# piotrmwojcik/GI-GS

Measured on AMD Instinct MI355X. Metric: train-step renders/sec (fwd+bwd, G-buffer+indirect) at 800x800; PSNR vs the CPU oracle, higher is better.
Workload: dtype f32; 1 GPU; C2 (configs[1] TensoIR lego stand-in): 300k surface Gaussians, 800x800, SH deg 2, GI step=16 start=8 delta=0.0625; P=300000, N=640000, M=9, hip_graphs=on, fused_glue=on, gi_march=proj, rasterizer=whole step = 2 hand-captured hipGraphs (fwd, bwd), asynchronous binning

## Files before the change

### gi-gs_amd/csrc/api.hip

```cpp
#include <cstdarg>
#include <cstdio>
#include <cstdlib>
#include <cstring>
#include <map>
#include <algorithm>
#include <new>
#include <mutex>
#include <vector>

#include "../../include/gigs_hip.h"
#include "gigs_common.h"

namespace {

thread_local char g_err[512] = "";

int fail(int code, const char* fmt, ...) {
  va_list ap;
  va_start(ap, fmt);
  vsnprintf(g_err, sizeof(g_err), fmt, ap);
  va_end(ap);
  return code;
}

// ... 70 lines not shown
  const char* ll = getenv("GIGS_LONG_LISTS");
  o.long_lists = (ll && ll[0]) ? (ll[0] == '1' ? 1 : 0) : -1;
  o.bucket_target = std::max(256, env_int("GIGS_BUCKET_TARGET", 1536));
  o.bin_bands = std::max(0, env_int("GIGS_BIN_BANDS", 0));
  o.blend_cull = env_int("GIGS_BLEND_CULL", 1) != 0;
  o.pre_bwd_sh_skip = env_int("GIGS_PRE_BWD_SH_SKIP", 1) != 0;
  o.gi_march = 4;
  if (const char* e = getenv("GIGS_GI_MARCH")) {
    if (strcmp(e, "exact") == 0) o.gi_march = 0;
  }
  o.gi_cert = env_int("GIGS_GI_CERT", 1) != 0;
  o.gi_interleave = env_int("GIGS_GI_INTERLEAVE", 1) != 0;
  o.gi_tile_log2w = env_int("GIGS_GI_TILE_LOG2W", 3);
  if (o.gi_tile_log2w < 0 || o.gi_tile_log2w > 6) o.gi_tile_log2w = 3;
  o.gi_zero_rays = env_int("GIGS_GI_ZERO_RAYS", 0) != 0;
  o.spec_max8 = env_int("GIGS_SPEC_MAX8", 128);
  o.spec_max16 = env_int("GIGS_SPEC_MAX16", 1500);
  o.shade_lds_floats = env_int("GIGS_SHADE_LDS_FLOATS", 30 * 1024);
  o.shade_bwd_blocks = std::max(0, env_int("GIGS_SHADE_BWD_BLOCKS", 0));
  o.shade_bwd_rows = env_int("GIGS_SHADE_BWD_ROWS", 0) != 0;
  o.spec_sparse = env_int("GIGS_SPEC_SPARSE", 1) != 0;
  o.spec_sparse_permille = env_int("GIGS_SPEC_SPARSE_PERMILLE", 37);
  if (o.spec_sparse_permille < 0 || o.spec_sparse_permille > 1000) o.spec_sparse_permille = 37;
  return o;
}
const gigs::Ctx& ctx_of(const gigs_ctx* c) { return c ? *reinterpret_cast<const gigs::Ctx*>(c) : gigs::default_ctx(); }

struct ProfRec { int stage; hipEvent_t a, b; };
std::mutex g_prof_mu;
bool g_prof_on = false;
std::vector<ProfRec> g_prof_recs;
std::vector<hipEvent_t> g_prof_pool;

hipEvent_t prof_event() {
  if (!g_prof_pool.empty()) {
    hipEvent_t e = g_prof_pool.back();
    g_prof_pool.pop_back();
    return e;
  }
  hipEvent_t e;
  hipEventCreate(&e);
  return e;
}

struct StageScope {
  hipStream_t s;
// ... 82 lines not shown
  gigs::ImageState s = gigs::ImageState::fromChunk(p, N, T);
  const void* ptrs[] = {s.final_T, s.n_contrib, s.ranges, s.tile_order};
  if (which < 0 || which >= 4) return -1;
  return (long long)((const char*)ptrs[which] - base);
}

gigs_ctx* gigs_ctx_create(void) {
  gigs::Ctx* c = new (std::nothrow) gigs::Ctx(gigs::default_ctx());
  if (!c) fail(GIGS_ERR_ALLOC, "gigs_ctx_create: out of host memory");
  return reinterpret_cast<gigs_ctx*>(c);
}
void gigs_ctx_destroy(gigs_ctx* ctx) { delete reinterpret_cast<gigs::Ctx*>(ctx); }

int gigs_ctx_get_options(const gigs_ctx* ctx, gigs_options* out) {
  if (!out || out->struct_bytes < (int)sizeof(gigs_options)) return fail(GIGS_ERR_INVALID, "gigs_ctx_get_options: set struct_bytes = sizeof(gigs_options)");
  const gigs::Options& o = ctx_of(ctx).opt;
  out->struct_bytes = (int)sizeof(gigs_options);
  out->binning_legacy = o.binning_legacy; out->bucket_max_mean = o.bucket_max_mean; out->long_lists = o.long_lists;
  out->bucket_target = o.bucket_target; out->bin_bands = o.bin_bands; out->blend_cull = o.blend_cull; out->pre_bwd_sh_skip = o.pre_bwd_sh_skip;
  out->gi_march = o.gi_march; out->gi_cert = o.gi_cert; out->gi_interleave = o.gi_interleave;
  out->gi_tile_log2w = o.gi_tile_log2w; out->gi_zero_rays = o.gi_zero_rays; out->spec_max8 = o.spec_max8;
  out->spec_max16 = o.spec_max16; out->shade_lds_floats = o.shade_lds_floats; out->shade_bwd_blocks = o.shade_bwd_blocks;
  out->shade_bwd_rows = o.shade_bwd_rows; out->spec_sparse = o.spec_sparse; out->spec_sparse_permille = o.spec_sparse_permille;
  return 0;
}
int gigs_ctx_set_options(gigs_ctx* ctx, const gigs_options* in) {
  if (!ctx) return fail(GIGS_ERR_INVALID, "gigs_ctx_set_options: the default context is immutable, create one");
  if (!in || in->struct_bytes < (int)sizeof(gigs_options)) return fail(GIGS_ERR_INVALID, "gigs_ctx_set_options: set struct_bytes = sizeof(gigs_options)");
  if (in->gi_march != 0 && in->gi_march != 4) return fail(GIGS_ERR_INVALID, "gi_march must be 0 (exact) or 4 (proj)");
  if (in->gi_tile_log2w < 0 || in->gi_tile_log2w > 6) return fail(GIGS_ERR_INVALID, "gi_tile_log2w must be 0..6");
  if (in->long_lists < -1 || in->long_lists > 1) return fail(GIGS_ERR_INVALID, "long_lists must be -1, 0 or 1");
  if (in->bucket_target < 256 || in->bucket_max_mean < 0 || in->bin_bands < 0 || in->bin_bands > 64)
    return fail(GIGS_ERR_INVALID, "bucket_target >= 256, bucket_max_mean >= 0, 0 <= bin_bands <= 64");
  if (in->spec_max8 < 0 || in->spec_max16 < in->spec_max8) return fail(GIGS_ERR_INVALID, "0 <= spec_max8 <= spec_max16");
  if (in->shade_lds_floats < 0 || in->shade_bwd_blocks < 0) return fail(GIGS_ERR_INVALID, "shade_lds_floats, shade_bwd_blocks >= 0");
  if (in->spec_sparse_permille < 0 || in->spec_sparse_permille > 1000) return fail(GIGS_ERR_INVALID, "0 <= spec_sparse_permille <= 1000");
  gigs::Options& o = reinterpret_cast<gigs::Ctx*>(ctx)->opt;
  o.binning_legacy = in->binning_legacy != 0; o.bucket_max_mean = in->bucket_max_mean; o.long_lists = in->long_lists;
  o.bucket_target = in->bucket_target; o.bin_bands = in->bin_bands; o.blend_cull = in->blend_cull != 0; o.pre_bwd_sh_skip = in->pre_bwd_sh_skip != 0;
  o.gi_march = in->gi_march; o.gi_cert = in->gi_cert != 0; o.gi_interleave = in->gi_interleave != 0;
  o.gi_tile_log2w = in->gi_tile_log2w; o.gi_zero_rays = in->gi_zero_rays != 0; o.spec_max8 = in->spec_max8;
  o.spec_max16 = in->spec_max16; o.shade_lds_floats = in->shade_lds_floats; o.shade_bwd_blocks = in->shade_bwd_blocks;
  o.shade_bwd_rows = in->shade_bwd_rows != 0; o.spec_sparse = in->spec_sparse != 0; o.spec_sparse_permille = in->spec_sparse_permille;
  return 0;
}
int gigs_ctx_set_reuse_binning(gigs_ctx* ctx, int on) {
  if (!ctx) return fail(GIGS_ERR_INVALID, "gigs_ctx_set_reuse_binning: the default context is immutable, create one");
  reinterpret_cast<gigs::Ctx*>(ctx)->reuse_binning = on != 0;
  return 0;
}
int gigs_ctx_set_split_sh(gigs_ctx* ctx, const float* sh_rest) {
  if (!ctx) return fail(GIGS_ERR_INVALID, "gigs_ctx_set_split_sh: the default context is immutable, create one");
  reinterpret_cast<gigs::Ctx*>(ctx)->sh_rest = sh_rest;
  return 0;
}
int gigs_ctx_set_materials_only(gigs_ctx* ctx, void* violations) {
  if (!ctx) return fail(GIGS_ERR_INVALID, "gigs_ctx_set_materials_only: the default context is immutable, create one");
  reinterpret_cast<gigs::Ctx*>(ctx)->materials_only = reinterpret_cast<unsigned*>(violations);
  return 0;
}
int gigs_ctx_set_blend_begin_event(gigs_ctx* ctx, void* hip_event) {
  if (!ctx) return fail(GIGS_ERR_INVALID, "gigs_ctx_set_blend_begin_event: the default context is immutable, create one");
  reinterpret_cast<gigs::Ctx*>(ctx)->blend_begin_event = hip_event;
  return 0;
}

// ... 499 lines not shown
```

### gi-gs_amd/csrc/gigs_common.h

```cpp
#pragma once
#include <hip/hip_runtime.h>
#include <stdint.h>

#define GIGS_BLOCK_X 16
#define GIGS_BLOCK_Y 16
#define GIGS_TILE (GIGS_BLOCK_X * GIGS_BLOCK_Y)
#define GIGS_BREC_F4 5
#define GIGS_GREC 20

namespace gigs {

struct v3 { float x, y, z; };
struct v4 { float x, y, z, w; };

__device__ __forceinline__ v3 operator+(v3 a, v3 b) { return {a.x + b.x, a.y + b.y, a.z + b.z}; }
__device__ __forceinline__ v3 operator-(v3 a, v3 b) { return {a.x - b.x, a.y - b.y, a.z - b.z}; }
__device__ __forceinline__ v3 operator*(v3 a, float s) { return {a.x * s, a.y * s, a.z * s}; }
__device__ __forceinline__ float dot3(v3 a, v3 b) { return a.x * b.x + a.y * b.y + a.z * b.z; }
__device__ __forceinline__ v3 cross3(v3 a, v3 b) {
  return {a.y * b.z - a.z * b.y, a.z * b.x - a.x * b.z, a.x * b.y - a.y * b.x};
}
__device__ __forceinline__ v3 normalize3(v3 v) {
  float inv = 1.0f / sqrtf(dot3(v, v));
  return v * inv;
// ... 164 lines not shown
  S::fromChunk(p, a...);
  return reinterpret_cast<size_t>(p) + kAlign;
}

struct Options {
  int binning_legacy;
  int bucket_max_mean;
  int long_lists;
  int bucket_target;
  int bin_bands;
  int blend_cull;
  int pre_bwd_sh_skip;
  int gi_march;
  int gi_cert;
  int gi_interleave;
  int gi_tile_log2w;
  int gi_zero_rays;
  int spec_max8, spec_max16;
  int shade_lds_floats;
  int shade_bwd_blocks;
  int shade_bwd_rows;
  int spec_sparse;
  int spec_sparse_permille;
};
struct Ctx {
  Options opt;
  unsigned async_capacity;
  unsigned* async_counters;
  void* blend_begin_event;
  int reuse_binning;
  unsigned* materials_only;
  const float* sh_rest;
};
const Options& default_options();
const Ctx& default_ctx();

struct FwdArgs {
  int P, D, M, W, H;
  unsigned gx, gy;
  float focal_x, focal_y, tan_fovx, tan_fovy, scale_modifier;
  const float *means3D, *shs, *colors_precomp, *opacities, *normal, *albedo, *roughness,
      *metallic, *scales, *rotations, *cov3D_precomp, *viewmatrix, *projmatrix, *cam_pos,
      *background;
  int argmax_depth, inference;
  const float* shs_rest;
};
// ... 72 lines not shown
```

### gi-gs_amd/csrc/pbr.hip

```cpp
#include <cmath>
#include <cstdlib>
#include <cstring>
#include <map>
#include <mutex>
#include <vector>

#include "gigs_common.h"
#include "pixel_ops.h"

namespace gigs {

__device__ __forceinline__ v3 safe_normalize(v3 v) {
  const float l = sqrtf(v.x * v.x + v.y * v.y + v.z * v.z);
  return l > 0.0f ? v3{v.x / l, v.y / l, v.z / l} : v3{0, 0, 0};
}
__device__ __forceinline__ v3 cube_dir_raw(float fx, float fy, int side) {
  switch (side) {
    case 0: return {1, -fy, -fx};
    case 1: return {-1, -fy, fx};
    case 2: return {fx, 1, fy};
    case 3: return {fx, -1, -fy};
    case 4: return {fx, -fy, 1};
    default: return {-fx, -fy, -1};
  }
// ... 252 lines not shown
      const int yy = (int)(((float)i + 0.5f) * inv), xx = i - yy * wd;
      const float w = W[(size_t)base + i];
      W2[(size_t)base + i] = w >= 0.0f ? w / divisor[(s * N + ymin + yy) * N + xmin + xx] : w;
    }
  }
}

typedef float pbr_f2 __attribute__((ext_vector_type(2)));

template <int kLanes>
__device__ __forceinline__ float group_sum_last(float v) {
  v += pbr_dpp<0xb1>(v);
  v += pbr_dpp<0x4e>(v);
  if (kLanes == 8) return v + pbr_dpp<0x141>(v);
  v += pbr_dpp<0x124>(v);
  v += pbr_dpp<0x128>(v);
  if (kLanes == 64) {
    v += pbr_dpp<0x142, 0xa>(v);
    v += pbr_dpp<0x143, 0xc>(v);
  }
  return v;
}

template <bool kBackward, bool kNorm, int kLanes>
__device__ __forceinline__ void specular_apply_body(int block, int N, const float* __restrict__ src,
                                                    const float* __restrict__ bounds, const uint32_t* __restrict__ offsets,
                                                    const float* __restrict__ W, float* __restrict__ dst,
                                                    float* __restrict__ wsum_out) {
  constexpr int kPerWave = 64 / kLanes;
  constexpr int kU = 4;
  const int lane = threadIdx.x & 63;
  const int total = 6 * N * N;
  const int o_raw = (block * 4 + (threadIdx.x >> 6)) * kPerWave + lane / kLanes;
  const bool valid = o_raw < total;
  const int o = valid ? o_raw : total - 1;
  const int g = lane % kLanes;
  const int stride = (kBackward && !kNorm) ? 4 : 3;

  __shared__ int face_tab[4 * kPerWave * 20];
  int* tab = face_tab + ((threadIdx.x >> 6) * kPerWave + lane / kLanes) * 20;
  const float4* b4 = reinterpret_cast<const float4*>(bounds + 24 * (size_t)o);
  const uint32_t first = offsets[6 * (size_t)o];
  int n_all;
  {
    int wd[6], pre[7], base[6];
    pre[0] = 0;
#pragma unroll
    for (int s = 0; s < 6; ++s) {
      const float4 b = b4[s];
      const int xmin = (int)b.x, xmax = (int)b.y, ymin = (int)b.z, ymax = (int)b.w;
      const bool empty = xmin > xmax || ymin > ymax;
      wd[s] = empty ? 1 : xmax - xmin + 1;
      pre[s + 1] = pre[s] + (empty ? 0 : wd[s] * (ymax - ymin + 1));
      base[s] = empty ? 0 : (s * N + ymin) * N + xmin;
    }
    n_all = pre[6];
    if (g == 0) {
#pragma unroll
      for (int s = 0; s < 7; ++s) tab[s] = pre[s];
#pragma unroll
      for (int s = 0; s < 6; ++s) { tab[8 + s] = wd[s]; tab[14 + s] = base[s]; }
    }
// ... 85 lines not shown
  float c0 = acc01.x, c1 = acc01.y, c2 = accw2.y, wsum = accw2.x;
  c0 = group_sum_last<kLanes>(c0); c1 = group_sum_last<kLanes>(c1); c2 = group_sum_last<kLanes>(c2);
  if (!kBackward) wsum = group_sum_last<kLanes>(wsum);
  if (g == kLanes - 1 && valid) {
    if (kBackward) {
      float* q = dst + 3 * (size_t)o;
      q[0] = c0; q[1] = c1; q[2] = c2;
    } else if (kNorm) {
      float* q = dst + 3 * (size_t)o;
      q[0] = c0 / wsum; q[1] = c1 / wsum; q[2] = c2 / wsum;
      wsum_out[o] = wsum;
    } else {
      float* q = dst + 4 * (size_t)o;
      q[0] = c0; q[1] = c1; q[2] = c2; q[3] = wsum;
    }
  }
}

template <bool kBackward, bool kNorm, int kLanes>
__global__ void __launch_bounds__(256)
specular_apply_kernel(int N, const float* __restrict__ src, const float* __restrict__ bounds,
                      const uint32_t* __restrict__ offsets, const float* __restrict__ W,
                      float* __restrict__ dst, float* __restrict__ wsum_out) {
  specular_apply_body<kBackward, kNorm, kLanes>(blockIdx.x, N, src, bounds, offsets, W, dst, wsum_out);
}

struct SpecLevel {
  int N, lanes, block_begin;
  const float* src;
  const float* bounds;
  const uint32_t* offsets;
  const float* W;
  float* dst;
  float* wsum_out;
};
struct SpecLevels { int n; SpecLevel lv[8]; };

template <bool kBackward>
__global__ void __launch_bounds__(256) specular_apply_multi_kernel(SpecLevels L) {
  int k = 0;
#pragma unroll
  for (int i = 1; i < 8; i++)
    if (i < L.n && (int)blockIdx.x >= L.lv[i].block_begin) k = i;
  const SpecLevel& v = L.lv[k];
  const int block = (int)blockIdx.x - v.block_begin;
  if (v.lanes == 8) specular_apply_body<kBackward, true, 8>(block, v.N, v.src, v.bounds, v.offsets, v.W, v.dst, v.wsum_out);
  else if (v.lanes == 16) specular_apply_body<kBackward, true, 16>(block, v.N, v.src, v.bounds, v.offsets, v.W, v.dst, v.wsum_out);
  else specular_apply_body<kBackward, true, 64>(block, v.N, v.src, v.bounds, v.offsets, v.W, v.dst, v.wsum_out);
}

static int spec_lanes_for(const Options& o, int avg_window) {
  return (avg_window > 0 && avg_window <= o.spec_max8) ? 8 : (avg_window > 0 && avg_window <= o.spec_max16) ? 16 : 64;
}

template <bool kBackward, bool kNorm>
static void launch_specular_apply(const Options& o, int res, int avg_window, const float* src, const float* bounds,
                                  const uint32_t* offsets, const float* W, float* dst, float* wsum_out, hipStream_t s) {
  const int total = 6 * res * res;
  const int max8 = o.spec_max8, max16 = o.spec_max16;
  if (avg_window > 0 && avg_window <= max8) {
    const int waves = (total + 7) / 8;
    hipLaunchKernelGGL((specular_apply_kernel<kBackward, kNorm, 8>), dim3((waves + 3) / 4), dim3(256), 0, s, res, src,
                       bounds, offsets, W, dst, wsum_out);
  } else if (avg_window > 0 && avg_window <= max16) {
    const int waves = (total + 3) / 4;
    hipLaunchKernelGGL((specular_apply_kernel<kBackward, kNorm, 16>), dim3((waves + 3) / 4), dim3(256), 0, s, res, src,
                       bounds, offsets, W, dst, wsum_out);
  } else {
    hipLaunchKernelGGL((specular_apply_kernel<kBackward, kNorm, 64>), dim3((total + 3) / 4), dim3(256), 0, s, res, src,
                       bounds, offsets, W, dst, wsum_out);
  }
}

struct SparseLevel {
  int total, cap, block_begin, group_begin, N;
  int vec;
  int chunks;
  int lds;
  const float* src;
  float* dst;
  const float* bounds;
  const uint32_t* offsets;
  const float* Wfwd;
  const float* wsum;
  int* list;
};
struct SparseLevels { int n; SparseLevel lv[8]; };

constexpr int kCensusPerThread = 4;

__global__ void __launch_bounds__(256) specular_census_kernel(SparseLevels L, int* __restrict__ state) {
  int k = 0;
#pragma unroll
  for (int i = 1; i < 8; i++)
    if (i < L.n && (int)blockIdx.x >= L.lv[i].block_begin) k = i;
  const SparseLevel& v = L.lv[k];
  const int lane = threadIdx.x & 63;
  const int t0 = (((int)blockIdx.x - v.block_begin) * 256 + (int)threadIdx.x) * kCensusPerThread;
  bool nz[kCensusPerThread];
  if (v.vec && t0 + kCensusPerThread <= v.total) {
    const float4* s4 = reinterpret_cast<const float4*>(v.src + 3 * (size_t)t0);
    float4* d4 = reinterpret_cast<float4*>(v.dst + 3 * (size_t)t0);
    const float4 a = s4[0], b = s4[1], c = s4[2];
    nz[0] = a.x != 0.0f || a.y != 0.0f || a.z != 0.0f;
    nz[1] = a.w != 0.0f || b.x != 0.0f || b.y != 0.0f;
    nz[2] = b.z != 0.0f || b.w != 0.0f || c.x != 0.0f;
    nz[3] = c.y != 0.0f || c.z != 0.0f || c.w != 0.0f;
    const float4 z = {0.0f, 0.0f, 0.0f, 0.0f};
    d4[0] = z; d4[1] = z; d4[2] = z;
  } else {
#pragma unroll
    for (int j = 0; j < kCensusPerThread; j++) {
      nz[j] = false;
      if (t0 + j < v.total) {
        const float* s = v.src + 3 * (size_t)(t0 + j);
        float* d = v.dst + 3 * (size_t)(t0 + j);
        nz[j] = s[0] != 0.0f || s[1] != 0.0f || s[2] != 0.0f;
        d[0] = 0.0f; d[1] = 0.0f; d[2] = 0.0f;
      }
    }
  }
  unsigned long long m[kCensusPerThread];
  int wave_total = 0;
#pragma unroll
  for (int j = 0; j < kCensusPerThread; j++) { m[j] = __ballot(nz[j]); wave_total += __popcll(m[j]); }
  __shared__ int wave_base[5];
  const int wave = threadIdx.x >> 6;
  if (lane == 0) wave_base[wave] = wave_total;
  __syncthreads();
  if (threadIdx.x == 0) {
    const int t01 = wave_base[0] + wave_base[1], t012 = t01 + wave_base[2], all = t012 + wave_base[3];
    const int first = all ? atomicAdd(state + k, all) : 0;
    wave_base[3] = first + t012; wave_base[2] = first + t01; wave_base[1] = first + wave_base[0]; wave_base[0] = first;
  }
  __syncthreads();
  if (wave_total == 0) return;
  int base = wave_base[wave];
  const unsigned long long below = (1ull << lane) - 1ull;
#pragma unroll
  for (int j = 0; j < kCensusPerThread; j++) {
    const int slot = base + __popcll(m[j] & below);
    if (nz[j] && slot < v.cap) v.list[slot] = t0 + j;
    base += __popcll(m[j]);
  }
}

constexpr int kScatterU = 2;
constexpr int kLdsTile = 32;
constexpr int kLdsParts = 8;
constexpr int kLdsWide = 16;

__global__ void __launch_bounds__(256) specular_scatter_kernel(SparseLevels L, int* __restrict__ state) {
  const int lane = threadIdx.x & 63;
  const int group = (int)blockIdx.x * 4 + ((int)threadIdx.x >> 6);
  if (blockIdx.x == 0 && threadIdx.x < 8 && (int)threadIdx.x < L.n) {
    const int c = state[threadIdx.x];
    state[8 + threadIdx.x] = c <= L.lv[threadIdx.x].cap ? 1 : 0;
    state[16 + threadIdx.x] = c;
  }
  int k = 0;
#pragma unroll
  for (int i = 1; i < 8; i++)
    if (i < L.n && group >= L.lv[i].group_begin) k = i;
  const SparseLevel& v = L.lv[k];
  const int count = state[k];
  if (count > v.cap) return;
  if (v.lds) {
    __shared__ float img[kLdsTile * kLdsTile * 3];
    const int N = v.N, nt = (N + kLdsTile - 1) / kLdsTile, bl = (group - v.group_begin) >> 2;
    const int face = bl % 6, tile = (bl / 6) % (nt * nt), part = bl / (6 * nt * nt);
    const int tx0 = (tile % nt) * kLdsTile, ty0 = (tile / nt) * kLdsTile;
    const int tx1 = min(tx0 + kLdsTile, N) - 1, ty1 = min(ty0 + kLdsTile, N) - 1;
    const int wave = (int)threadIdx.x >> 6;
    for (int i = threadIdx.x; i < kLdsTile * kLdsTile * 3; i += 256) img[i] = 0.0f;
    __syncthreads();
    const int listed = min(count, v.cap);
    for (int slot = part + kLdsParts * wave; slot < listed; slot += kLdsParts * 4) {
      const int o = __builtin_amdgcn_readfirstlane(v.list[slot]);
      const float4* b4 = reinterpret_cast<const float4*>(v.bounds + 24 * (size_t)o);
      int before = 0, xmin = 0, xmax = -1, ymin = 0, ymax = -1;
#pragma unroll
      for (int s = 0; s < 6; ++s) {
        const float4 b = b4[s];
        const int x0 = (int)b.x, x1 = (int)b.y, y0 = (int)b.z, y1 = (int)b.w;
        const int cnt = (x0 > x1 || y0 > y1) ? 0 : (x1 - x0 + 1) * (y1 - y0 + 1);
        if (s < face) before += cnt;
        if (s == face && cnt) { xmin = x0; xmax = x1; ymin = y0; ymax = y1; }
      }
      const int ix0 = max(xmin, tx0), ix1 = min(xmax, tx1), iy0 = max(ymin, ty0), iy1 = min(ymax, ty1);
      if (ix0 > ix1 || iy0 > iy1) continue;
      const int wd = xmax - xmin + 1, iw = ix1 - ix0 + 1, ni = iw * (iy1 - iy0 + 1);
// ... 6 lines not shown
        const float w = W[(y - ymin) * wd + (x - xmin)];
        if (!(w >= 0.0f)) continue;
        float* t = img + 3 * ((y - ty0) * kLdsTile + (x - tx0));
        const float q = w / ws;
        const float v0 = q * g0, v1 = q * g1, v2 = q * g2;
        if (v0 != 0.0f) atomicAdd(t, v0);
        if (v1 != 0.0f) atomicAdd(t + 1, v1);
        if (v2 != 0.0f) atomicAdd(t + 2, v2);
      }
    }
    __syncthreads();
    const int row3 = 3 * (tx1 - tx0 + 1), cells = row3 * (ty1 - ty0 + 1);
    for (int i = threadIdx.x; i < cells; i += 256) {
      const int yy = i / row3, xc = i - yy * row3;
      const float val = img[3 * yy * kLdsTile + xc];
      if (val != 0.0f) atomicAdd(v.dst + 3 * ((size_t)(face * N + ty0 + yy) * N + tx0) + xc, val);
    }
    return;
  }
  const int slot = (group - v.group_begin) / v.chunks, chunk = (group - v.group_begin) % v.chunks;
  if (slot >= count || slot >= v.cap) return;
  const int o = __builtin_amdgcn_readfirstlane(v.list[slot]);
  const int N = v.N;
  int pre[7], wd[6], base[6];
  float inv[6];
  pre[0] = 0;
  const float4* b4 = reinterpret_cast<const float4*>(v.bounds + 24 * (size_t)o);
#pragma unroll
  for (int s = 0; s < 6; ++s) {
    const float4 b = b4[s];
    const int xmin = (int)b.x, xmax = (int)b.y, ymin = (int)b.z, ymax = (int)b.w;
    const bool empty = xmin > xmax || ymin > ymax;
    wd[s] = empty ? 1 : xmax - xmin + 1;
    inv[s] = 1.0f / (float)wd[s];
    pre[s + 1] = pre[s] + (empty ? 0 : wd[s] * (ymax - ymin + 1));
    base[s] = empty ? 0 : (s * N + ymin) * N + xmin;
  }
  const int n = pre[6];
  const float* W = v.Wfwd + v.offsets[6 * (size_t)o];
  const float ws = v.wsum[o];
  const float* g = v.src + 3 * (size_t)o;
  const float g0 = g[0], g1 = g[1], g2 = g[2];
  const int step = 64 * v.chunks;
  int from[3];
  float gch[3];
#pragma unroll
  for (int j = 0; j < 3; j++) {
    const int D = 64 * j + lane, ch = D % 3;
    from[j] = D / 3;
    gch[j] = ch == 0 ? g0 : ch == 1 ? g1 : g2;
  }
  const int ch0 = lane % 3;
  for (int c0 = 64 * chunk; c0 < n; c0 += step * kScatterU) {
    float w[kScatterU];
#pragma unroll
    for (int u = 0; u < kScatterU; u++) {
      const int c = c0 + u * step + lane;
      w[u] = c < n ? W[c] : -1.0f;
    }
#pragma unroll
    for (int u = 0; u < kScatterU; u++) {
      if (c0 + u * step >= n) break;
      const int c = c0 + u * step + lane;
      float q = -1.0f;
      int texel = 0;
      if (w[u] >= 0.0f) {
        int f = 0;
#pragma unroll
        for (int j = 1; j < 6; j++) f += c >= pre[j] ? 1 : 0;
        int f_pre = pre[0], f_wd = wd[0], f_base = base[0];
        float f_inv = inv[0];
#pragma unroll
        for (int j = 1; j < 6; j++)
          if (f == j) { f_pre = pre[j]; f_wd = wd[j]; f_base = base[j]; f_inv = inv[j]; }
        const int loc = c - f_pre;
        const int row = (int)(((float)loc + 0.5f) * f_inv);
        texel = f_base + row * N + (loc - row * f_wd);
        q = w[u] / ws;
      }
#pragma unroll
      for (int j = 0; j < 3; j++) {
        const float qq = __shfl(q, from[j]);
        const int tt = __shfl(texel, from[j]);
        const int ch = ch0 + j >= 3 ? ch0 + j - 3 : ch0 + j;
        const float val = qq * gch[j];
        if (!(qq < 0.0f) && val != 0.0f) atomicAdd(v.dst + 3 * (size_t)tt + ch, val);
      }
    }
  }
}

__global__ void __launch_bounds__(256) specular_apply_multi_bwd_sparse_kernel(SpecLevels L, int* __restrict__ state) {
  int k = 0;
#pragma unroll
  for (int i = 1; i < 8; i++)
    if (i < L.n && (int)blockIdx.x >= L.lv[i].block_begin) k = i;
  if (blockIdx.x == 0 && threadIdx.x < 8) state[threadIdx.x] = 0;
  if (state[8 + k] != 0) return;
  const SpecLevel& v = L.lv[k];
  const int block = (int)blockIdx.x - v.block_begin;
  if (v.lanes == 8) specular_apply_body<true, true, 8>(block, v.N, v.src, v.bounds, v.offsets, v.W, v.dst, v.wsum_out);
  else if (v.lanes == 16) specular_apply_body<true, true, 16>(block, v.N, v.src, v.bounds, v.offsets, v.W, v.dst, v.wsum_out);
  else specular_apply_body<true, true, 64>(block, v.N, v.src, v.bounds, v.offsets, v.W, v.dst, v.wsum_out);
}

static int spec_sparse_capacity(const Options& o, int res) {
  return (int)((long long)6 * res * res * o.spec_sparse_permille / 1000);
}

__device__ __forceinline__ int cube_face_uv(float x, float y, float z, float& u, float& v) {
  const float ax = fabsf(x), ay = fabsf(y), az = fabsf(z);
  int idx;
  float c;
  if (az > fmaxf(ax, ay)) { idx = 4; c = z; }
  else if (ay > ax) { idx = 2; c = y; y = z; }
  else { idx = 0; c = x; x = z; }
  if (c < 0.f) idx += 1;
  const float m = (1.0f / fabsf(c)) * 0.5f;
  const float m0 = (idx == 0 || idx == 5) ? -m : m;
  const float m1 = (idx != 2) ? -m : m;
  u = x * m0 + 0.5f;
  v = y * m1 + 0.5f;
  if (!isfinite(u) || !isfinite(v)) return -1;
  u = fminf(fmaxf(u, 0.f), 1.f);
  v = fminf(fmaxf(v, 0.f), 1.f);
  return idx;
// ... 823 lines not shown
  void* tok; gigs_internal_stage_begin(backward ? 17 : 16, stream, &tok);
  if (backward) hipLaunchKernelGGL(gigs::specular_apply_multi_kernel<true>, dim3(blocks), dim3(256), 0, (hipStream_t)stream, L);
  else hipLaunchKernelGGL(gigs::specular_apply_multi_kernel<false>, dim3(blocks), dim3(256), 0, (hipStream_t)stream, L);
  gigs_internal_stage_end(tok);
  PBR_CHECK_LAUNCH();
  return 0;
}

int gigs_spec_sparse_capacity(const gigs_ctx* ctx, int res) {
  if (res <= 0 || res > 4096) return gigs_internal_fail(GIGS_ERR_INVALID, "spec_sparse_capacity: bad resolution");
  return gigs::spec_sparse_capacity(*gigs_internal_options(ctx), res);
}

int gigs_specular_cubemap_multi_bwd_sparse(gigs_ctx* ctx, int n_levels, const gigs_spec_level* levels,
                                           const float* const* weights_fwd, const float* const* wsum, int* state,
                                           int* lists, void* stream) {
  const gigs::Options& o = *gigs_internal_options(ctx);
  if (!o.spec_sparse) return gigs_specular_cubemap_multi_w(ctx, n_levels, levels, 1, stream);
  if (n_levels <= 0 || n_levels > 8 || !levels || !weights_fwd || !wsum || !state || !lists)
    return gigs_internal_fail(GIGS_ERR_INVALID, "specular_cubemap_multi_bwd_sparse: bad argument");
  gigs::SpecLevels L;
  gigs::SparseLevels S;
  L.n = S.n = n_levels;
  int blocks = 0, census_blocks = 0, groups = 0;
  size_t list_begin = 0;
  for (int i = 0; i < n_levels; i++) {
    const gigs_spec_level& a = levels[i];
    if (a.res <= 0 || a.res > 4096 || !a.src || !a.bounds || !a.offsets || !a.weights || !a.dst || !weights_fwd[i] || !wsum[i])
      return gigs_internal_fail(GIGS_ERR_INVALID, "specular_cubemap_multi_bwd_sparse: bad level");
    gigs::SpecLevel& v = L.lv[i];
    v.N = a.res; v.lanes = gigs::spec_lanes_for(o, a.avg_window); v.block_begin = blocks;
    v.src = a.src; v.bounds = a.bounds; v.offsets = a.offsets; v.W = a.weights; v.dst = a.dst; v.wsum_out = a.wsum;
    const int total = 6 * a.res * a.res;
    const int waves = v.lanes == 64 ? total : (total + (64 / v.lanes) - 1) / (64 / v.lanes);
    blocks += (waves + 3) / 4;
    gigs::SparseLevel& q = S.lv[i];
    q.total = total; q.cap = gigs::spec_sparse_capacity(o, a.res); q.block_begin = census_blocks; q.group_begin = groups; q.N = a.res;
    q.vec = ((((uintptr_t)a.src) | ((uintptr_t)a.dst)) & 15) == 0;
    q.src = a.src; q.dst = a.dst; q.bounds = a.bounds; q.offsets = a.offsets; q.Wfwd = weights_fwd[i]; q.wsum = wsum[i];
    q.list = lists + list_begin;
    const int per_block = 256 * gigs::kCensusPerThread;
    census_blocks += (total + per_block - 1) / per_block;
    q.chunks = std::min(32, std::max(1, (std::max(1, a.avg_window) + 64 * 2 * gigs::kScatterU - 1) / (64 * 2 * gigs::kScatterU)));
    q.lds = (long long)a.avg_window * gigs::kLdsWide >= total;
    const int nt = (a.res + gigs::kLdsTile - 1) / gigs::kLdsTile;
    groups += q.lds ? 4 * 6 * nt * nt * gigs::kLdsParts : (q.cap * q.chunks + 3) / 4 * 4;
    list_begin += (size_t)q.cap;
  }
  hipStream_t s = (hipStream_t)stream;
  void* tok; gigs_internal_stage_begin(17, stream, &tok);
  hipLaunchKernelGGL(gigs::specular_census_kernel, dim3(census_blocks), dim3(256), 0, s, S, state);
  hipLaunchKernelGGL(gigs::specular_scatter_kernel, dim3(std::max(1, (groups + 3) / 4)), dim3(256), 0, s, S, state);
  hipLaunchKernelGGL(gigs::specular_apply_multi_bwd_sparse_kernel, dim3(blocks), dim3(256), 0, s, L, state);
  gigs_internal_stage_end(tok);
  PBR_CHECK_LAUNCH();
  return 0;
}

int gigs_cubemap_mip_fwd(int res_out, int channels, const float* in, float* out, void* stream) {
  if (res_out <= 0 || channels <= 0 || !in || !out) return gigs_internal_fail(GIGS_ERR_INVALID, "cubemap_mip_fwd: bad argument");
  void* tok; gigs_internal_stage_begin(16, stream, &tok);
  hipLaunchKernelGGL(gigs::cubemap_mip_fwd_kernel, dim3((6 * res_out * res_out * channels + 255) / 256), dim3(256), 0, (hipStream_t)stream, res_out, channels, in, out);
  gigs_internal_stage_end(tok);
  PBR_CHECK_LAUNCH();
  return 0;
}

int gigs_cubemap_mip_bwd(int res_out, const float* dout, float* din, void* stream) {
  if (res_out <= 0 || !dout || !din) return gigs_internal_fail(GIGS_ERR_INVALID, "cubemap_mip_bwd: bad argument");
  const int res = 2 * res_out;
  void* tok; gigs_internal_stage_begin(17, stream, &tok);
  hipLaunchKernelGGL(gigs::cubemap_mip_bwd_kernel, dim3((6 * res * res + 255) / 256), dim3(256), 0, (hipStream_t)stream, res_out, dout, din, (const float*)nullptr,
                     (const float*)nullptr);
  gigs_internal_stage_end(tok);
  PBR_CHECK_LAUNCH();
  return 0;
// ... 273 lines not shown
```

### gi-gs_amd/gigs_lib.py

```python
from __future__ import annotations

import ctypes as C
import functools
import os
import threading

_HERE = os.path.dirname(os.path.abspath(__file__))
LIB_PATH = os.environ.get("GIGS_LIB", os.path.join(_HERE, "libgigs_hip.so"))

ALLOC_FN = C.CFUNCTYPE(C.c_void_p, C.c_size_t, C.c_void_p)

_f = C.c_void_p
_i = C.c_int
_fl = C.c_float

SIGNATURES = {
    "gigs_last_error": (C.c_char_p, []),
    "gigs_build_arch": (C.c_char_p, []),
    "gigs_required_geom": (C.c_size_t, [_i]),
    "gigs_required_image": (C.c_size_t, [_i, _i]),
    "gigs_required_binning": (C.c_size_t, [_i]),
    "gigs_forward": (_i, [C.c_void_p, ALLOC_FN, C.c_void_p, ALLOC_FN, C.c_void_p, ALLOC_FN, C.c_void_p,
                          _i, _i, _i, _f, _i, _i,
                          _f, _f, _f, _f, _f, _f, _f, _f,
# ... 119 lines not shown
    "gigs_stream_delay": (_i, [C.c_uint, C.c_void_p]),
    "gigs_ctx_set_async_binning": (_i, [C.c_void_p, _i, C.c_void_p]),
    "gigs_ctx_create": (C.c_void_p, []),
    "gigs_ctx_destroy": (None, [C.c_void_p]),
    "gigs_ctx_get_options": (_i, [C.c_void_p, C.c_void_p]),
    "gigs_ctx_set_options": (_i, [C.c_void_p, C.c_void_p]),
    "gigs_profile_begin": (None, []),
    "gigs_profile_end": (_i, [C.POINTER(C.c_float), C.POINTER(C.c_int), _i]),
    "gigs_profile_stage_name": (C.c_char_p, [_i]),
}

class ShadeExt(C.Structure):
    _fields_ = [("planar", C.c_int), ("rough_scale", C.c_float), ("rough_bias", C.c_float),
                ("out_F0", C.c_void_p), ("out_linear", C.c_void_p), ("out_roughness", C.c_void_p),
                ("g_albedo_mul_a", C.c_void_p), ("g_albedo_mul_b", C.c_void_p),
                ("g_roughness_add", C.c_void_p), ("g_metallic_add", C.c_void_p),
                ("g_scale", C.c_void_p), ("lamb_mask", C.c_void_p), ("lamb_acc4", C.c_void_p)]


class Options(C.Structure):
    _fields_ = [(n, C.c_int) for n in (
        "struct_bytes", "binning_legacy", "bucket_max_mean", "long_lists", "bucket_target", "bin_bands", "blend_cull",
        "pre_bwd_sh_skip", "gi_march", "gi_cert", "gi_interleave", "gi_tile_log2w", "gi_zero_rays", "spec_max8",
        "spec_max16", "shade_lds_floats", "shade_bwd_blocks", "shade_bwd_rows", "spec_sparse", "spec_sparse_permille")]


OPTION_NAMES = tuple(n for n, _ in Options._fields_ if n != "struct_bytes")
GI_MARCHES = {0: "exact", 4: "proj"}
_GI_MARCH_VALUES = {name: value for value, name in GI_MARCHES.items()}


class SpecLevel(C.Structure):
    _fields_ = [("res", C.c_int), ("avg_window", C.c_int), ("src", C.c_void_p), ("bounds", C.c_void_p),
                ("offsets", C.c_void_p), ("weights", C.c_void_p), ("dst", C.c_void_p), ("wsum", C.c_void_p)]


class AdamGroup(C.Structure):
    _fields_ = [("param", C.c_void_p), ("grad", C.c_void_p), ("exp_avg", C.c_void_p), ("exp_avg_sq", C.c_void_p),
                ("n", C.c_longlong), ("lr", C.c_double), ("step", C.c_int)]


class ActivationRaw(C.Structure):
    _fields_ = [(n, C.c_void_p) for n in ("f_dc", "f_rest", "opacity", "normal", "albedo", "roughness", "metallic",
                                          "scaling", "rotation")]


class ActivationOut(C.Structure):
# ... 221 lines not shown
```

### include/gigs_hip.h

```cpp
#ifndef GIGS_HIP_H_
#define GIGS_HIP_H_

#include <stddef.h>
#include <stdint.h>

#ifdef __cplusplus
extern "C" {
#endif

#define GIGS_OK 0
#define GIGS_ERR_INVALID (-1)
#define GIGS_ERR_HIP (-2)
#define GIGS_ERR_ALLOC (-3)

typedef char* (*gigs_alloc_fn)(size_t nbytes, void* user);

const char* gigs_last_error(void);
const char* gigs_build_arch(void);

typedef struct gigs_ctx gigs_ctx;
typedef struct gigs_options {
  int struct_bytes;
  int binning_legacy;
  int bucket_max_mean;
  int long_lists;
  int bucket_target;
  int bin_bands;
  int blend_cull;
  int pre_bwd_sh_skip;
  int gi_march;
  int gi_cert;
  int gi_interleave;
  int gi_tile_log2w;
  int gi_zero_rays;
  int spec_max8;
  int spec_max16;
  int shade_lds_floats;
  int shade_bwd_blocks;
  int shade_bwd_rows;
  int spec_sparse;
  int spec_sparse_permille;
} gigs_options;
gigs_ctx* gigs_ctx_create(void);
void gigs_ctx_destroy(gigs_ctx* ctx);
int gigs_ctx_get_options(const gigs_ctx* ctx, gigs_options* out);
int gigs_ctx_set_options(gigs_ctx* ctx, const gigs_options* in);

size_t gigs_required_geom(int P);
size_t gigs_required_image(int width, int height);
size_t gigs_required_binning(int num_rendered);

int gigs_forward(gigs_ctx* ctx, gigs_alloc_fn geometryBuffer, void* geom_user, gigs_alloc_fn binningBuffer,
                 void* binning_user, gigs_alloc_fn imageBuffer, void* image_user, int P, int D, int M,
                 const float* background, int width, int height, const float* means3D,
                 const float* shs, const float* colors_precomp, const float* opacities,
                 const float* normal, const float* albedo, const float* roughness,
                 const float* metallic, const float* scales, float scale_modifier,
                 const float* rotations, const float* cov3D_precomp, const float* viewmatrix,
                 const float* projmatrix, const float* cam_pos, float tan_fovx, float tan_fovy,
                 int prefiltered, int argmax_depth, int inference, float* out_color,
                 float* out_opacity, float* out_depth, float* out_normal, float* out_normal_view,
                 float* out_pos, float* out_albedo, float* out_roughness, float* out_metallic,
                 int* radii, int debug, void* stream);

// ... 317 lines not shown
```

Baseline: 353.9 renders/s.

## Fuse sparse specular scatter and dense backward apply into one launch

The backward sparse specular path drops from three kernels to two. The census kernel now finalises the per-level sparse/dense decision through a last-block ticket atomic. A single fused kernel then runs both the sparse scatter groups and the dense apply blocks, each block skipping itself according to that decision. Scatter groups are reordered so LDS-tiled levels come first, and the per-object face table moves from registers into LDS. The fused path is on by default and guarded by an option. It removes one launch and its serialisation point, at the cost of a larger shared LDS buffer and a grid that holds both block types.

```diff
diff --git a/gi-gs_amd/csrc/api.hip b/gi-gs_amd/csrc/api.hip
--- a/gi-gs_amd/csrc/api.hip
+++ b/gi-gs_amd/csrc/api.hip
@@ -116,6 +116,7 @@
   o.spec_sparse = env_int("GIGS_SPEC_SPARSE", 1) != 0;
   o.spec_sparse_permille = env_int("GIGS_SPEC_SPARSE_PERMILLE", 37);
   if (o.spec_sparse_permille < 0 || o.spec_sparse_permille > 1000) o.spec_sparse_permille = 37;
+  o.spec_sparse_fused = env_int("GIGS_SPEC_SPARSE_FUSED", 1) != 0;
   return o;
 }
 const gigs::Ctx& ctx_of(const gigs_ctx* c) { return c ? *reinterpret_cast<const gigs::Ctx*>(c) : gigs::default_ctx(); }
@@ -244,6 +245,7 @@
   out->gi_tile_log2w = o.gi_tile_log2w; out->gi_zero_rays = o.gi_zero_rays; out->spec_max8 = o.spec_max8;
   out->spec_max16 = o.spec_max16; out->shade_lds_floats = o.shade_lds_floats; out->shade_bwd_blocks = o.shade_bwd_blocks;
   out->shade_bwd_rows = o.shade_bwd_rows; out->spec_sparse = o.spec_sparse; out->spec_sparse_permille = o.spec_sparse_permille;
+  out->spec_sparse_fused = o.spec_sparse_fused;
   return 0;
 }
 int gigs_ctx_set_options(gigs_ctx* ctx, const gigs_options* in) {
@@ -264,6 +266,7 @@
   o.gi_tile_log2w = in->gi_tile_log2w; o.gi_zero_rays = in->gi_zero_rays != 0; o.spec_max8 = in->spec_max8;
   o.spec_max16 = in->spec_max16; o.shade_lds_floats = in->shade_lds_floats; o.shade_bwd_blocks = in->shade_bwd_blocks;
   o.shade_bwd_rows = in->shade_bwd_rows != 0; o.spec_sparse = in->spec_sparse != 0; o.spec_sparse_permille = in->spec_sparse_permille;
+  o.spec_sparse_fused = in->spec_sparse_fused != 0;
   return 0;
 }
 int gigs_ctx_set_reuse_binning(gigs_ctx* ctx, int on) {
diff --git a/gi-gs_amd/csrc/gigs_common.h b/gi-gs_amd/csrc/gigs_common.h
--- a/gi-gs_amd/csrc/gigs_common.h
+++ b/gi-gs_amd/csrc/gigs_common.h
@@ -210,6 +210,7 @@
   int shade_bwd_rows;
   int spec_sparse;
   int spec_sparse_permille;
+  int spec_sparse_fused;
 };
 struct Ctx {
   Options opt;
diff --git a/gi-gs_amd/csrc/pbr.hip b/gi-gs_amd/csrc/pbr.hip
--- a/gi-gs_amd/csrc/pbr.hip
+++ b/gi-gs_amd/csrc/pbr.hip
@@ -298,11 +298,13 @@
   return v;
 }
 
+constexpr int kFaceTabInts(int lanes) { return 4 * (64 / lanes) * 20; }
+
 template <bool kBackward, bool kNorm, int kLanes>
 __device__ __forceinline__ void specular_apply_body(int block, int N, const float* __restrict__ src,
                                                     const float* __restrict__ bounds, const uint32_t* __restrict__ offsets,
                                                     const float* __restrict__ W, float* __restrict__ dst,
-                                                    float* __restrict__ wsum_out) {
+                                                    float* __restrict__ wsum_out, int* face_tab) {
   constexpr int kPerWave = 64 / kLanes;
   constexpr int kU = 4;
   const int lane = threadIdx.x & 63;
@@ -313,7 +315,6 @@
   const int g = lane % kLanes;
   const int stride = (kBackward && !kNorm) ? 4 : 3;
 
-  __shared__ int face_tab[4 * kPerWave * 20];
   int* tab = face_tab + ((threadIdx.x >> 6) * kPerWave + lane / kLanes) * 20;
   const float4* b4 = reinterpret_cast<const float4*>(bounds + 24 * (size_t)o);
   const uint32_t first = offsets[6 * (size_t)o];
@@ -445,7 +446,8 @@
 specular_apply_kernel(int N, const float* __restrict__ src, const float* __restrict__ bounds,
                       const uint32_t* __restrict__ offsets, const float* __restrict__ W,
                       float* __restrict__ dst, float* __restrict__ wsum_out) {
-  specular_apply_body<kBackward, kNorm, kLanes>(blockIdx.x, N, src, bounds, offsets, W, dst, wsum_out);
+  __shared__ int face_tab[kFaceTabInts(kLanes)];
+  specular_apply_body<kBackward, kNorm, kLanes>(blockIdx.x, N, src, bounds, offsets, W, dst, wsum_out, face_tab);
 }
 
 struct SpecLevel {
@@ -460,16 +462,20 @@
 struct SpecLevels { int n; SpecLevel lv[8]; };
 
 template <bool kBackward>
+__device__ __forceinline__ void specular_apply_level(const SpecLevel& v, int block, int* face_tab) {
+  if (v.lanes == 8) specular_apply_body<kBackward, true, 8>(block, v.N, v.src, v.bounds, v.offsets, v.W, v.dst, v.wsum_out, face_tab);
+  else if (v.lanes == 16) specular_apply_body<kBackward, true, 16>(block, v.N, v.src, v.bounds, v.offsets, v.W, v.dst, v.wsum_out, face_tab);
+  else specular_apply_body<kBackward, true, 64>(block, v.N, v.src, v.bounds, v.offsets, v.W, v.dst, v.wsum_out, face_tab);
+}
+
+template <bool kBackward>
 __global__ void __launch_bounds__(256) specular_apply_multi_kernel(SpecLevels L) {
   int k = 0;
 #pragma unroll
   for (int i = 1; i < 8; i++)
     if (i < L.n && (int)blockIdx.x >= L.lv[i].block_begin) k = i;
-  const SpecLevel& v = L.lv[k];
-  const int block = (int)blockIdx.x - v.block_begin;
-  if (v.lanes == 8) specular_apply_body<kBackward, true, 8>(block, v.N, v.src, v.bounds, v.offsets, v.W, v.dst, v.wsum_out);
-  else if (v.lanes == 16) specular_apply_body<kBackward, true, 16>(block, v.N, v.src, v.bounds, v.offsets, v.W, v.dst, v.wsum_out);
-  else specular_apply_body<kBackward, true, 64>(block, v.N, v.src, v.bounds, v.offsets, v.W, v.dst, v.wsum_out);
+  __shared__ int face_tab[kFaceTabInts(8)];
+  specular_apply_level<kBackward>(L.lv[k], (int)blockIdx.x - L.lv[k].block_begin, face_tab);
 }
 
 static int spec_lanes_for(const Options& o, int avg_window) {
@@ -496,7 +502,8 @@
 }
 
 struct SparseLevel {
-  int total, cap, block_begin, group_begin, N;
+  int total, cap, block_begin, N;
+  int group_begin, group_end;
   int vec;
   int chunks;
   int lds;
@@ -512,6 +519,9 @@
 
 constexpr int kCensusPerThread = 4;
 
+constexpr int kSparseTicket = 24;
+
+template <bool kFinish>
 __global__ void __launch_bounds__(256) specular_census_kernel(SparseLevels L, int* __restrict__ state) {
   int k = 0;
 #pragma unroll
@@ -555,6 +565,20 @@
     const int t01 = wave_base[0] + wave_base[1], t012 = t01 + wave_base[2], all = t012 + wave_base[3];
     const int first = all ? atomicAdd(state + k, all) : 0;
     wave_base[3] = first + t012; wave_base[2] = first + t01; wave_base[1] = first + wave_base[0]; wave_base[0] = first;
+    int one = 1;
+    asm volatile("" : "+v"(one) : "v"(first));
+    if (kFinish && __hip_atomic_fetch_add(state + kSparseTicket, one, __ATOMIC_RELAXED, __HIP_MEMORY_SCOPE_AGENT) == (int)gridDim.x - 1) {
+#pragma unroll
+      for (int l = 0; l < 8; l++) {
+        if (l < L.n) {
+          const int c = __hip_atomic_load(state + l, __ATOMIC_RELAXED, __HIP_MEMORY_SCOPE_AGENT);
+          state[8 + l] = c <= L.lv[l].cap ? 1 : 0;
+          state[16 + l] = c;
+        }
+        state[l] = 0;
+      }
+      state[kSparseTicket] = 0;
+    }
   }
   __syncthreads();
   if (wave_total == 0) return;
@@ -572,24 +596,22 @@
 constexpr int kLdsTile = 32;
 constexpr int kLdsParts = 8;
 constexpr int kLdsWide = 16;
-
-__global__ void __launch_bounds__(256) specular_scatter_kernel(SparseLevels L, int* __restrict__ state) {
+constexpr int kSparseLdsFloats = kLdsTile * kLdsTile * 3;
+constexpr int kScatterTabInts = 32;
+static_assert(kFaceTabInts(8) <= kSparseLdsFloats && 4 * kScatterTabInts <= kSparseLdsFloats, "one buffer for every body");
+
+__device__ __forceinline__ int scatter_level_of(const SparseLevels& L, int group) {
+  int k = -1;
+#pragma unroll
+  for (int i = 0; i < 8; i++)
+    if (i < L.n && group >= L.lv[i].group_begin && group < L.lv[i].group_end) k = i;
+  return k;
+}
+
+__device__ __forceinline__ void specular_scatter_body(const SparseLevel& v, int group, int count, float* lds) {
   const int lane = threadIdx.x & 63;
-  const int group = (int)blockIdx.x * 4 + ((int)threadIdx.x >> 6);
-  if (blockIdx.x == 0 && threadIdx.x < 8 && (int)threadIdx.x < L.n) {
-    const int c = state[threadIdx.x];
-    state[8 + threadIdx.x] = c <= L.lv[threadIdx.x].cap ? 1 : 0;
-    state[16 + threadIdx.x] = c;
-  }
-  int k = 0;
-#pragma unroll
-  for (int i = 1; i < 8; i++)
-    if (i < L.n && group >= L.lv[i].group_begin) k = i;
-  const SparseLevel& v = L.lv[k];
-  const int count = state[k];
-  if (count > v.cap) return;
   if (v.lds) {
-    __shared__ float img[kLdsTile * kLdsTile * 3];
+    float* img = lds;
     const int N = v.N, nt = (N + kLdsTile - 1) / kLdsTile, bl = (group - v.group_begin) >> 2;
     const int face = bl % 6, tile = (bl / 6) % (nt * nt), part = bl / (6 * nt * nt);
     const int tx0 = (tile % nt) * kLdsTile, ty0 = (tile / nt) * kLdsTile;
@@ -642,21 +664,29 @@
   if (slot >= count || slot >= v.cap) return;
   const int o = __builtin_amdgcn_readfirstlane(v.list[slot]);
   const int N = v.N;
-  int pre[7], wd[6], base[6];
-  float inv[6];
-  pre[0] = 0;
-  const float4* b4 = reinterpret_cast<const float4*>(v.bounds + 24 * (size_t)o);
-#pragma unroll
-  for (int s = 0; s < 6; ++s) {
-    const float4 b = b4[s];
-    const int xmin = (int)b.x, xmax = (int)b.y, ymin = (int)b.z, ymax = (int)b.w;
-    const bool empty = xmin > xmax || ymin > ymax;
-    wd[s] = empty ? 1 : xmax - xmin + 1;
-    inv[s] = 1.0f / (float)wd[s];
-    pre[s + 1] = pre[s] + (empty ? 0 : wd[s] * (ymax - ymin + 1));
-    base[s] = empty ? 0 : (s * N + ymin) * N + xmin;
-  }
-  const int n = pre[6];
+  int* tab = reinterpret_cast<int*>(lds) + ((int)threadIdx.x >> 6) * kScatterTabInts;
+  int n;
+  {
+    int pre = 0;
+    const float4* b4 = reinterpret_cast<const float4*>(v.bounds + 24 * (size_t)o);
+#pragma unroll
+    for (int s = 0; s < 6; ++s) {
+      const float4 b = b4[s];
+      const int xmin = (int)b.x, xmax = (int)b.y, ymin = (int)b.z, ymax = (int)b.w;
+      const bool empty = xmin > xmax || ymin > ymax;
+      const int wd = empty ? 1 : xmax - xmin + 1;
+      if (lane == 0) {
+        tab[s] = pre; tab[8 + s] = wd; tab[14 + s] = empty ? 0 : (s * N + ymin) * N + xmin;
+        tab[20 + s] = __float_as_int(1.0f / (float)wd);
+      }
+      pre += empty ? 0 : wd * (ymax - ymin + 1);
+    }
+    n = pre;
+    if (lane == 0) tab[6] = n;
+    __builtin_amdgcn_fence(__ATOMIC_RELEASE, "wavefront");
+    __builtin_amdgcn_wave_barrier();
+    __builtin_amdgcn_fence(__ATOMIC_ACQUIRE, "wavefront");
+  }
   const float* W = v.Wfwd + v.offsets[6 * (size_t)o];
   const float ws = v.wsum[o];
   const float* g = v.src + 3 * (size_t)o;
@@ -687,15 +717,11 @@
       if (w[u] >= 0.0f) {
         int f = 0;
 #pragma unroll
-        for (int j = 1; j < 6; j++) f += c >= pre[j] ? 1 : 0;
-        int f_pre = pre[0], f_wd = wd[0], f_base = base[0];
-        float f_inv = inv[0];
-#pragma unroll
-        for (int j = 1; j < 6; j++)
-          if (f == j) { f_pre = pre[j]; f_wd = wd[j]; f_base = base[j]; f_inv = inv[j]; }
-        const int loc = c - f_pre;
-        const int row = (int)(((float)loc + 0.5f) * f_inv);
-        texel = f_base + row * N + (loc - row * f_wd);
+        for (int j = 1; j < 6; j++) f += c >= tab[j] ? 1 : 0;
+        const int f_wd = tab[8 + f];
+        const int loc = c - tab[f];
+        const int row = (int)(((float)loc + 0.5f) * __int_as_float(tab[20 + f]));
+        texel = tab[14 + f] + row * N + (loc - row * f_wd);
         q = w[u] / ws;
       }
 #pragma unroll
@@ -710,6 +736,22 @@
   }
 }
 
+__global__ void __launch_bounds__(256) specular_scatter_kernel(SparseLevels L, int* __restrict__ state) {
+  __shared__ float lds[kSparseLdsFloats];
+  if (blockIdx.x == 0 && threadIdx.x < 8 && (int)threadIdx.x < L.n) {
+    const int c = state[threadIdx.x];
+    state[8 + threadIdx.x] = c <= L.lv[threadIdx.x].cap ? 1 : 0;
+    state[16 + threadIdx.x] = c;
+  }
+  const int group = (int)blockIdx.x * 4 + ((int)threadIdx.x >> 6);
+  const int k = scatter_level_of(L, group);
+  if (k < 0) return;
+  const SparseLevel& v = L.lv[k];
+  const int count = state[k];
+  if (count > v.cap) return;
+  specular_scatter_body(v, group, count, lds);
+}
+
 __global__ void __launch_bounds__(256) specular_apply_multi_bwd_sparse_kernel(SpecLevels L, int* __restrict__ state) {
   int k = 0;
 #pragma unroll
@@ -717,11 +759,27 @@
     if (i < L.n && (int)blockIdx.x >= L.lv[i].block_begin) k = i;
   if (blockIdx.x == 0 && threadIdx.x < 8) state[threadIdx.x] = 0;
   if (state[8 + k] != 0) return;
-  const SpecLevel& v = L.lv[k];
-  const int block = (int)blockIdx.x - v.block_begin;
-  if (v.lanes == 8) specular_apply_body<true, true, 8>(block, v.N, v.src, v.bounds, v.offsets, v.W, v.dst, v.wsum_out);
-  else if (v.lanes == 16) specular_apply_body<true, true, 16>(block, v.N, v.src, v.bounds, v.offsets, v.W, v.dst, v.wsum_out);
-  else specular_apply_body<true, true, 64>(block, v.N, v.src, v.bounds, v.offsets, v.W, v.dst, v.wsum_out);
+  __shared__ int face_tab[kFaceTabInts(8)];
+  specular_apply_level<true>(L.lv[k], (int)blockIdx.x - L.lv[k].block_begin, face_tab);
+}
+
+__global__ void __launch_bounds__(256) specular_bwd_sparse_fused_kernel(SparseLevels S, SpecLevels L, int scatter_blocks,
+                                                                        const int* __restrict__ state) {
+  __shared__ float lds[kSparseLdsFloats];
+  if ((int)blockIdx.x < scatter_blocks) {
+    const int group = (int)blockIdx.x * 4 + ((int)threadIdx.x >> 6);
+    const int k = scatter_level_of(S, group);
+    if (k < 0 || state[8 + k] == 0) return;
+    specular_scatter_body(S.lv[k], group, state[16 + k], lds);
+  } else {
+    const int b = (int)blockIdx.x - scatter_blocks;
+    int k = 0;
+#pragma unroll
+    for (int i = 1; i < 8; i++)
+      if (i < L.n && b >= L.lv[i].block_begin) k = i;
+    if (state[8 + k] != 0) return;
+    specular_apply_level<true>(L.lv[k], b - L.lv[k].block_begin, reinterpret_cast<int*>(lds));
+  }
 }
 
 static int spec_sparse_capacity(const Options& o, int res) {
@@ -1591,7 +1649,7 @@
   gigs::SpecLevels L;
   gigs::SparseLevels S;
   L.n = S.n = n_levels;
-  int blocks = 0, census_blocks = 0, groups = 0;
+  int blocks = 0, census_blocks = 0;
   size_t list_begin = 0;
   for (int i = 0; i < n_levels; i++) {
     const gigs_spec_level& a = levels[i];
@@ -1604,7 +1662,7 @@
     const int waves = v.lanes == 64 ? total : (total + (64 / v.lanes) - 1) / (64 / v.lanes);
     blocks += (waves + 3) / 4;
     gigs::SparseLevel& q = S.lv[i];
-    q.total = total; q.cap = gigs::spec_sparse_capacity(o, a.res); q.block_begin = census_blocks; q.group_begin = groups; q.N = a.res;
+    q.total = total; q.cap = gigs::spec_sparse_capacity(o, a.res); q.block_begin = census_blocks; q.N = a.res;
     q.vec = ((((uintptr_t)a.src) | ((uintptr_t)a.dst)) & 15) == 0;
     q.src = a.src; q.dst = a.dst; q.bounds = a.bounds; q.offsets = a.offsets; q.Wfwd = weights_fwd[i]; q.wsum = wsum[i];
     q.list = lists + list_begin;
@@ -1612,15 +1670,29 @@
     census_blocks += (total + per_block - 1) / per_block;
     q.chunks = std::min(32, std::max(1, (std::max(1, a.avg_window) + 64 * 2 * gigs::kScatterU - 1) / (64 * 2 * gigs::kScatterU)));
     q.lds = (long long)a.avg_window * gigs::kLdsWide >= total;
-    const int nt = (a.res + gigs::kLdsTile - 1) / gigs::kLdsTile;
-    groups += q.lds ? 4 * 6 * nt * nt * gigs::kLdsParts : (q.cap * q.chunks + 3) / 4 * 4;
     list_begin += (size_t)q.cap;
   }
+  int groups = 0;
+  for (int pass = 0; pass < 2; pass++)
+    for (int i = 0; i < n_levels; i++) {
+      gigs::SparseLevel& q = S.lv[i];
+      if (o.spec_sparse_fused ? (q.lds != 0) != (pass == 0) : pass != 0) continue;
+      const int nt = (q.N + gigs::kLdsTile - 1) / gigs::kLdsTile;
+      q.group_begin = groups;
+      groups += q.lds ? 4 * 6 * nt * nt * gigs::kLdsParts : (q.cap * q.chunks + 3) / 4 * 4;
+      q.group_end = groups;
+    }
   hipStream_t s = (hipStream_t)stream;
   void* tok; gigs_internal_stage_begin(17, stream, &tok);
-  hipLaunchKernelGGL(gigs::specular_census_kernel, dim3(census_blocks), dim3(256), 0, s, S, state);
-  hipLaunchKernelGGL(gigs::specular_scatter_kernel, dim3(std::max(1, (groups + 3) / 4)), dim3(256), 0, s, S, state);
-  hipLaunchKernelGGL(gigs::specular_apply_multi_bwd_sparse_kernel, dim3(blocks), dim3(256), 0, s, L, state);
+  if (o.spec_sparse_fused) {
+    hipLaunchKernelGGL(gigs::specular_census_kernel<true>, dim3(census_blocks), dim3(256), 0, s, S, state);
+    hipLaunchKernelGGL(gigs::specular_bwd_sparse_fused_kernel, dim3(groups / 4 + blocks), dim3(256), 0, s, S, L, groups / 4,
+                       (const int*)state);
+  } else {
+    hipLaunchKernelGGL(gigs::specular_census_kernel<false>, dim3(census_blocks), dim3(256), 0, s, S, state);
+    hipLaunchKernelGGL(gigs::specular_scatter_kernel, dim3(std::max(1, groups / 4)), dim3(256), 0, s, S, state);
+    hipLaunchKernelGGL(gigs::specular_apply_multi_bwd_sparse_kernel, dim3(blocks), dim3(256), 0, s, L, state);
+  }
   gigs_internal_stage_end(tok);
   PBR_CHECK_LAUNCH();
   return 0;
diff --git a/gi-gs_amd/gigs_lib.py b/gi-gs_amd/gigs_lib.py
--- a/gi-gs_amd/gigs_lib.py
+++ b/gi-gs_amd/gigs_lib.py
@@ -165,7 +165,8 @@
     _fields_ = [(n, C.c_int) for n in (
         "struct_bytes", "binning_legacy", "bucket_max_mean", "long_lists", "bucket_target", "bin_bands", "blend_cull",
         "pre_bwd_sh_skip", "gi_march", "gi_cert", "gi_interleave", "gi_tile_log2w", "gi_zero_rays", "spec_max8",
-        "spec_max16", "shade_lds_floats", "shade_bwd_blocks", "shade_bwd_rows", "spec_sparse", "spec_sparse_permille")]
+        "spec_max16", "shade_lds_floats", "shade_bwd_blocks", "shade_bwd_rows", "spec_sparse", "spec_sparse_permille",
+        "spec_sparse_fused")]
 
 
 OPTION_NAMES = tuple(n for n, _ in Options._fields_ if n != "struct_bytes")
diff --git a/include/gigs_hip.h b/include/gigs_hip.h
--- a/include/gigs_hip.h
+++ b/include/gigs_hip.h
@@ -40,6 +40,7 @@
   int shade_bwd_rows;
   int spec_sparse;
   int spec_sparse_permille;
+  int spec_sparse_fused;
 } gigs_options;
 gigs_ctx* gigs_ctx_create(void);
 void gigs_ctx_destroy(gigs_ctx* ctx);
```

New measurement: 353.6 renders/s. About the same (-0.1%).
